# twmitchel/FieldConv

Measured on AMD Instinct MI355X. Metric: FieldConv fwd+bwd Medges/s (20k verts, k=32, C=48, M=2), higher is better.
Workload: dtype f32 (complex64 in/out; contractions on f16 MFMA with every operand split into two halves, fp32 accumulate)

## Files before the change

fieldconv_amd/_env.py:

```python
import os

SWITCHES = {
    'FC_MFMA': 'f32: fp32-MFMA contractions throughout; f16: single halves (reduced precision); default: split halves',
    'FC_RING': '0: frequency-major forward kernels for every mesh size; 2: ring-major ones for every size',
    'FC_GROUP_SPLIT': '0: the backward data kernel never runs the two frequency groups of a tile as separate work items; 2 (development): wherever legal',
    'FC_RING_COMPACT': '0: no compact LDS plans (aliased partials, half-size record chunks) for the ring-major forward kernel',
    'FC_RING_HALVES': '0: no half tiles in the last round of the ring-major forward kernel',
    'FC_HALF_TILES': '0: no half tiles in the frequency-major kernels; 2: half tiles in the backward kernels too',
    'FC_BWD_STREAM': '0: the data / filter kernel pair on large meshes too, instead of the H-streaming arrangement (gather + stream + gx kernels)',
    'FC_FILTER2': '0: the LDS-staged half-precision filter-gradient kernel instead of the register-fed one',
    'FC_SPLIT_FINISH': '1: partial sums and parameter-gradient chain as two launches',
    'FC_EDGE_PARTS_MAX': 'cap (log2) on the number of workgroups that share a tile on small meshes',
    'FC_ECHO_WPV': 'wavefronts per vertex in the ECHO descriptor kernels (1, 2 or 4)',
    'FC_STAMP_KERNEL': 'data | filter | stream: which backward kernel writes in-kernel time stamps (tools/stamps.py)',
    'FC_DEBUG': 'forward kernels: skip phases (WRONG RESULTS; refused by bench.py)',
    'FC_DEBUG_BWD': 'backward kernels: skip phases (bit 0 walk, bit 1 gxt product, bit 2 gW product, bit 3 H stores) (WRONG RESULTS; refused by bench.py)',
    'FC_LIN_DIRECT': '0: TangentLin on small meshes through the LDS-staged kernel instead of the direct one',
    'FC_DEBUG_RG': "ECHOBlock head's grouped GEMM: 1 no products, 2 no loads, 4 no staging (WRONG RESULTS; refused by bench.py)",
    'FC_DEBUG_RP': 'finishing launch: 1 no partial loads, 2 no parameter-gradient chain (WRONG RESULTS; refused by bench.py)',
    'FIELDCONV_DEV': '1: load libfieldconv_hip_dev.so (the library switches above exist there only; one of them set without this raises)',
    'FIELDCONV_HIP_LIB': 'path of a prebuilt libfieldconv_hip.so (development variants, fieldconv_amd.build.build_variant)',
    'FIELDCONV_DENSE': '1: FCPrecomp stencils through the dense-stencil kernels',
    'FIELDCONV_NO_GEO': '1: 64-byte factored records in the forward pass instead of geometric ones',
    'FIELDCONV_TORCH_GRAPH': '1: support graph built with torch ops instead of fc_graph_build',
    'FIELDCONV_NO_EDGE_SPLIT': '1: no edge split on small meshes',
    'FIELDCONV_EAGER_STENCIL': '1: FCPrecomp returns the dense (E,R,F) tensor',
    'FIELDCONV_NO_FUSED_EPILOGUE': '1: residual add and modReLU as separate operators',
    'FIELDCONV_SEPARATE_CALLS': '1: one foreign call per kernel instead of fc_forward_params / fc_backward_all',
    'FIELDCONV_CPP_NODES': '0: the block-level autograd nodes in Python (fieldconv_amd/blocks.py) instead of the C++ ones (fc_torch_nodes.so)',
    'FIELDCONV_ECHO_TAIL': "0: ECHOBlock's dense tail as torch's own Linear / ReLU autograd nodes instead of one node; aten: one node composed "
                           "of ATen GEMMs instead of the native head (fc_echo_head_*)",
    'FIELDCONV_BLOCK_CALLS': '0: FCResNetBlock / ECHOBlock / LiftBlock composed of per-operator autograd nodes instead of the block-level entry points',
    'BENCH_BACKEND': 'gloo: several ranks share a device (test rigs); default nccl (= RCCL)',
    'BENCH_FORCE_DIST': '1: run the partitioned / data-parallel code path with one rank',
    'BENCH_FORWARD_OVERLAP': '1: interior targets under the forward halo exchange',
    'BENCH_NO_OVERLAP': '1: gradient halo exchange not overlapped with the filter-gradient kernel',
    'BENCH_GRAPH_STEP': '1: the partitioned step captured in one HIP graph',
}

TEST_SWITCHES = {
    'FC_FULL_MODES': '1: tests/test_gpu_modes.py sweeps every development switch instead of the eight kernel-family / arithmetic modes',
    'FC_FUZZ_SHAPES': 'number of shapes in the seeded sweep against the oracle (default 40)',
    'FC_FUZZ_SEED': 'seed of that sweep',
    'FC_FUZZ_WIDE': '1: the sweep also draws layers wider than 64 channels and (n_rings, band_limit) pairs outside the compiled set',
    'FC_DIST_TEST_DEVICE': 'cuda: the distributed test worker runs the HIP kernels (two gloo ranks on one GPU)',
    'FC_DIST_OVERLAP': '0: the distributed test worker without forward / backward overlap',
    'FC_DIST_PLAN_ONLY': '1: the distributed test worker checks partition and halo plan at config-4 size only',
    'FC_DIST_CONFIG4': '1: the distributed GPU test worker runs config 4\'s per-rank size (20 000 owned vertices per rank)',
}

LIBRARY_SWITCHES = ('FC_BWD_STREAM', 'FC_RING', 'FC_GROUP_SPLIT', 'FC_RING_COMPACT', 'FC_RING_HALVES', 'FC_HALF_TILES', 'FC_FILTER2', 'FC_SPLIT_FINISH',
                    'FC_EDGE_PARTS_MAX', 'FC_ECHO_WPV', 'FC_STAMP_KERNEL', 'FC_DEBUG', 'FC_DEBUG_BWD', 'FC_DEBUG_RP', 'FC_DEBUG_RG', 'FC_LIN_DIRECT')

PREFIXES = ('FC_', 'FIELDCONV_', 'BENCH_')
WRONG_RESULTS = ('FC_DEBUG', 'FC_DEBUG_BWD', 'FC_DEBUG_RP', 'FC_DEBUG_RG')


def active(environ=None):
    environ = os.environ if environ is None else environ
    return {k: environ[k] for k in sorted(SWITCHES) if k in environ}


def unknown(environ=None):
    environ = os.environ if environ is None else environ
    return sorted(k for k in environ if k.startswith(PREFIXES) and k not in SWITCHES and k not in TEST_SWITCHES)
```

fieldconv_amd/csrc/fc_backward.hip:

```cpp
#include <stdio.h>
#include "fc_backward_kernels.hpp"
#include "fc_backward_stream.hpp"

namespace fc {

template <int T>
__global__ __launch_bounds__(kThreads) void fc_backward_filter_kernel(
    const float2* __restrict__ gx_, const float* __restrict__ hdump, float2* __restrict__ ggwp ,
    const BwdArgs a, const int F, const int B) {
    extern __shared__ __attribute__((aligned(16))) char smem[];
    const MmaGeom& mg = a.g;
    const int KD = a.KD, KP = mg.KP, IP = mg.MP, I = a.I;
    float* const slab0 = reinterpret_cast<float*>(smem);
    float* const xtr = slab0 + 2 * a.slab_stride;
    float* const xts = xtr + IP * kXtStride;
    float* const xtd = xts + IP * kXtStride;

    const int tid = threadIdx.x;
    const int lane = tid & 63;
    const int wave = __builtin_amdgcn_readfirstlane(tid >> 6);
    const int f = blockIdx.y;
    const int m = f - B;
    const int fr = lane & 15, fq = lane >> 4;

// ... 424 lines not shown
            if ((a.dbg & 32) && wave < mg.NMT) {
                const lds_f16* arow = img + fr * KSI + 8 * fq;
                const lds_f16* brow = img0 + (buf ^ 1) * kTile * KSI + fr * KSI + 8 * fq;
                f32x4 xr = {0.f, 0.f, 0.f, 0.f}, xi = xr;
                for (int kb = 0; kb < KP / 32; ++kb) {
                    const u32x4 arh = *reinterpret_cast<lds_u32x4*>(arow + kb * 32), arl = *reinterpret_cast<lds_u32x4*>(arow + kb * 32 + KP);
                    const u32x4 aih = *reinterpret_cast<lds_u32x4*>(arow + kb * 32 + 2 * KP), ail = *reinterpret_cast<lds_u32x4*>(arow + kb * 32 + 3 * KP);
                    const u32x4 brh = *reinterpret_cast<lds_u32x4*>(brow + kb * 32), brl = *reinterpret_cast<lds_u32x4*>(brow + kb * 32 + KP);
                    const u32x4 bih = *reinterpret_cast<lds_u32x4*>(brow + kb * 32 + 2 * KP), bil = *reinterpret_cast<lds_u32x4*>(brow + kb * 32 + 3 * KP);
                    xr = mfma32h(arh, brh, xr); xr = mfma32h(arh, brl, xr); xr = mfma32h(arl, brh, xr);
                    xr = mfma32h(aih, bih, xr); xr = mfma32h(aih, bil, xr); xr = mfma32h(ail, bih, xr);
                    xi = mfma32h(aih, brh, xi); xi = mfma32h(aih, brl, xi); xi = mfma32h(ail, brh, xi);
                    xi = mfma32h(arh, bih, xi); xi = mfma32h(arh, bil, xi); xi = mfma32h(arl, bih, xi);
                }
                const size_t cap = (size_t)gridDim.x * F * KP * IP;
                const size_t base = (((size_t)tile * F + f) * mg.NMT + wave) * 256 % (cap - 256);
#pragma unroll
                for (int jj = 0; jj < 4; ++jj) ggwp[base + (4 * fq + jj) * 16 + fr] = make_float2(xr[jj] * it, xi[jj] * it);
            }
        }
    
    };
    int buf = 0;
    for (int tile = blockIdx.x; tile < a.ntiles; tile += tile_step, buf ^= 1) {
        one_tile(tile, ahead0, buf);
        stamp(3);
    }
    stamp(30);
    stamp.realtime(31);

#pragma unroll
    for (int n = 0; n < T; ++n) {
        if (gw_h[n] >= 0) {
#pragma unroll
            for (int jj = 0; jj < 4; ++jj) {
                const int k = gw_h[n] + 4 * fq + jj;
                const int i = i0 + fr;
                ggwp[(((size_t)blockIdx.x * F + f) * KP + k) * IP + i] = make_float2(gre[n][jj], gim[n][jj]);
            }
        }
    }
}

__global__ void fc_reduce_gw_kernel(const float2* __restrict__ gwp, float2* __restrict__ gw, int P, int F, int R,
                                    int O, int I, int KP, int IP, int pairs ) {
    const int idx = blockIdx.x * blockDim.x + threadIdx.x;
    const int total = F * R * O * I;
    if (idx >= total) return;
    const int i = idx % I;
    const int k = (idx / I) % (R * O);
    const int f = idx / (I * R * O);
    float2 s = make_float2(0.f, 0.f);
    const size_t stride = (size_t)F * KP * IP;
    const float2* src = gwp + ((size_t)f * KP + k) * IP + i;
    int p = 0;
    for (; p + 8 <= P; p += 8) {
        float2 v[8];
#pragma unroll
        for (int u = 0; u < 8; ++u) v[u] = src[(size_t)(p + u) * stride];
#pragma unroll
        for (int u = 0; u < 8; ++u) { s.x += v[u].x; s.y += v[u].y; }
    }
    for (; p < P; ++p) {
        const float2 v = src[(size_t)p * stride];
        s.x += v.x;
        s.y += v.y;
    }
    const float sc = 1.f / (float)F;
    int r = k / O, o = k - r * O;
    if (pairs == 2) {
        o = k / R;
        r = k - o * R;
    } else if (pairs && k < (R >> 1) * 2 * O) {
        const int pr = k / (2 * O), rem = k - pr * 2 * O;
        r = 2 * pr + (rem & 1);
        o = rem >> 1;
    }
    gw[(((size_t)o * I + i) * R + r) * F + f] = make_float2(s.x * sc, s.y * sc);
}

template <int R, int B>
static int launch_gather(const float2* gy, const float* rec, const fc_csr* g, const float* wpk, char* hrec, const StreamArgs& a,
                         const StreamPlan& p, hipStream_t stream) {
    auto kern = fc_backward_gather_kernel<R, B>;
    const size_t lds = (size_t)kWaves * kRingChunks * 1024;
    const int grid = p.ntiles < num_cus() ? p.ntiles : num_cus();
    hipLaunchKernelGGL(kern, dim3(grid), dim3(kThreads), lds, stream, gy, rec, g->rowptr, g->runs, wpk, hrec, a);
    return hipGetLastError() == hipSuccess ? FC_OK : FC_ERR_LAUNCH;
}

template <int T, int KPT = 0, int IT = 0>
static int launch_stream(const float2* x, const char* hrec, const float* wpk, float2* gwp, float2* gxt, const StreamArgs& a,
                         const StreamPlan& p, hipStream_t stream) {
    auto kern = fc_backward_stream_kernel<T, KPT, IT>;
    static bool lds_ok[kMaxDevices] = {};
    if (!allow_full_lds(reinterpret_cast<const void*>(kern), p.lds, lds_ok)) return FC_ERR_LAUNCH;
    hipLaunchKernelGGL(kern, dim3(p.P, p.FS), dim3(kThreads), p.lds, stream, x, hrec, wpk, gwp, gxt, a);
    return hipGetLastError() == hipSuccess ? FC_OK : FC_ERR_LAUNCH;
}

int backward_stream_impl(const float* x, const float* gy, const float* rec, const fc_csr* g, const float* wpk, float* gx, void* ws,
                         size_t ws_bytes, const fc_dims* d, hipStream_t stream, int stages) {
    const StreamPlan p = plan_stream(d, halves_of(d), true);
    if (!p.ok) return FC_ERR_UNSUPPORTED;
    if (!ws || ws_bytes < p.hrec_bytes + p.gwp_bytes + p.gxt_bytes + p.wst_bytes) return FC_ERR_WORKSPACE;
    StreamArgs a = make_stream_args(d, p);
    char* hrec = static_cast<char*>(ws);
    a.wst = reinterpret_cast<uint32_t*>(hrec + p.hrec_bytes + p.gwp_bytes + p.gxt_bytes);
    float2* gwp = reinterpret_cast<float2*>(hrec + p.hrec_bytes);
    float2* gxt = reinterpret_cast<float2*>(hrec + p.hrec_bytes + p.gwp_bytes);
    const float2* x2 = reinterpret_cast<const float2*>(x);
    int rc = FC_ERR_UNSUPPORTED;
    if (stages & 1) {
        const float2* gy2 = reinterpret_cast<const float2*>(gy);
#define FC_GATHER_CASE(RR, BB) if (d->R == RR && d->B == BB) rc = launch_gather<RR, BB>(gy2, rec, g, wpk, hrec, a, p, stream);
        FC_GATHER_CASE(2, 1) FC_GATHER_CASE(4, 1) FC_GATHER_CASE(6, 1) FC_GATHER_CASE(8, 1)
        FC_GATHER_CASE(2, 2) FC_GATHER_CASE(4, 2) FC_GATHER_CASE(6, 2) FC_GATHER_CASE(8, 2)
        FC_GATHER_CASE(2, 3) FC_GATHER_CASE(4, 3) FC_GATHER_CASE(6, 3) FC_GATHER_CASE(8, 3)
#undef FC_GATHER_CASE
        if (rc != FC_OK) return rc;
    }
    if (!(stages & 2)) return FC_OK;
    if (p.T == 6 && p.KPS == 288 && d->I == 48) rc = launch_stream<6, 288, 48>(x2, hrec, wpk, gwp, gxt, a, p, stream);
    else if (p.T == 6 && p.KPS == 192 && d->I == 64) rc = launch_stream<6, 192, 64>(x2, hrec, wpk, gwp, gxt, a, p, stream);
    else if (p.T <= 2) rc = launch_stream<2>(x2, hrec, wpk, gwp, gxt, a, p, stream);
    else if (p.T <= 4) rc = launch_stream<4>(x2, hrec, wpk, gwp, gxt, a, p, stream);
    else rc = launch_stream<6>(x2, hrec, wpk, gwp, gxt, a, p, stream);
    if (rc != FC_OK || (stages & 4)) return rc;
    const size_t count = (size_t)d->N * d->I;
    const dim3 grid((unsigned)((count + 255) / 256));
    float2* gx2 = reinterpret_cast<float2*>(gx);
    if (d->B == 1) hipLaunchKernelGGL(fc_backward_gx_kernel<1>, grid, dim3(256), 0, stream, x2, gxt, gx2, count, p.KS);
    else if (d->B == 2) hipLaunchKernelGGL(fc_backward_gx_kernel<2>, grid, dim3(256), 0, stream, x2, gxt, gx2, count, p.KS);
    else hipLaunchKernelGGL(fc_backward_gx_kernel<3>, grid, dim3(256), 0, stream, x2, gxt, gx2, count, p.KS);
    return hipGetLastError() == hipSuccess ? FC_OK : FC_ERR_LAUNCH;
}

bool backward_streams(const fc_dims* d, bool factored) { return plan_stream(d, halves_of(d), factored).ok; }

bool backward_fits(const fc_dims* d) { return plan_backward(d, halves_of(d)).ok_factored; }

size_t backward_workspace_bytes(const fc_dims* d) {
    const BwdPlan p = plan_backward(d, halves_of(d));
    const size_t pair = p.hdump_bytes + p.gwp_bytes + p.gxp_bytes + 256;
    const StreamPlan sp = plan_stream(d, halves_of(d), true);
    const size_t stream = sp.ok ? sp.hrec_bytes + sp.gwp_bytes + sp.gxt_bytes + sp.wst_bytes + 256 : 0;
    return pair > stream ? pair : stream;
}

template <int T>
static int launch_backward_filter(const float2* x, const float* hdump, float2* gwp, const BwdArgs& a, const BwdPlan& p,
                                  const fc_dims* d, hipStream_t stream) {
    static const bool half2 = !(dev_env("FC_FILTER2") && atoi(dev_env("FC_FILTER2")) == 0);
    static bool ok_half2[kMaxDevices] = {}, ok_half[kMaxDevices] = {}, ok_f32[kMaxDevices] = {};
    if (p.fhalf && half2) {
        const size_t lds2 = (size_t)(2 * kTile * filter_image_stride(p.KP) + 2 * 6 * p.IP * kXbStride + 8) * sizeof(_Float16) + 16;
        static bool ok_half2h[kMaxDevices] = {};
        if (a.dump_halves) {
            if (!allow_full_lds(reinterpret_cast<const void*>(fc_backward_filter_half2_kernel<T, true>), lds2, ok_half2h)) return FC_ERR_LAUNCH;
            hipLaunchKernelGGL((fc_backward_filter_half2_kernel<T, true>), dim3(p.P, p.F), dim3(kThreads), lds2, stream, x, hdump, gwp, a, p.F,
                               d->B, d->R * d->O);
        } else {
            if (!allow_full_lds(reinterpret_cast<const void*>(fc_backward_filter_half2_kernel<T, false>), lds2, ok_half2)) return FC_ERR_LAUNCH;
            hipLaunchKernelGGL((fc_backward_filter_half2_kernel<T, false>), dim3(p.P, p.F), dim3(kThreads), lds2, stream, x, hdump, gwp, a, p.F,
                               d->B, d->R * d->O);
        }
    } else if (p.fhalf) {
        if (!allow_full_lds(reinterpret_cast<const void*>(fc_backward_filter_half_kernel<T>), p.lds_filter, ok_half)) return FC_ERR_LAUNCH;
        hipLaunchKernelGGL(fc_backward_filter_half_kernel<T>, dim3(p.P, p.F), dim3(kThreads), p.lds_filter, stream, x, hdump, gwp, a,
                           p.F, d->B, d->R * d->O);
    } else {
        if (!allow_full_lds(reinterpret_cast<const void*>(fc_backward_filter_kernel<T>), p.lds_filter, ok_f32)) return FC_ERR_LAUNCH;
        hipLaunchKernelGGL(fc_backward_filter_kernel<T>, dim3(p.P, p.F), dim3(kThreads), p.lds_filter, stream, x, hdump, gwp, a, p.F,
                           d->B);
    }
    return hipGetLastError() == hipSuccess ? FC_OK : FC_ERR_LAUNCH;
}

int backward_filter_impl(const float* x, void* ws, size_t ws_bytes, const fc_dims* d, hipStream_t stream, bool factored) {
    if (backward_streams(d, factored)) return FC_OK;
    const BwdPlan p = plan_backward(d, halves_of(d));
    if (!p.ok) return FC_ERR_UNSUPPORTED;
    if (!ws || ws_bytes < p.hdump_bytes + p.gwp_bytes) return FC_ERR_WORKSPACE;
    const BwdArgs a = make_args(d, p);
    const float* hdump = reinterpret_cast<const float*>(ws);
    float2* gwp = reinterpret_cast<float2*>(static_cast<char*>(ws) + p.hdump_bytes);
    const float2* x2 = reinterpret_cast<const float2*>(x);
    int need = (p.ngw + kWaves - 1) / kWaves;
    if (p.fhalf) {
        const int per_col = kWaves / p.g.NMT, row_tiles = p.KP / 16;
        need = (row_tiles + per_col - 1) / per_col;
    }
    if (need <= 2) return launch_backward_filter<2>(x2, hdump, gwp, a, p, d, stream);
    if (need <= 4) return launch_backward_filter<4>(x2, hdump, gwp, a, p, d, stream);
    if (need <= 6) return launch_backward_filter<6>(x2, hdump, gwp, a, p, d, stream);
    if (need <= kMaxGwTiles) return launch_backward_filter<kMaxGwTiles>(x2, hdump, gwp, a, p, d, stream);
    return FC_ERR_UNSUPPORTED;
}

void describe_backward(const fc_dims* d, int records, char* buf, size_t n) {
    {
        const StreamPlan sp = plan_stream(d, halves_of(d), records != 0);
        if (sp.ok) {
            snprintf(buf, n, "fc_backward_gather_kernel<records,split-f16> tiles=%d; fc_backward_stream_kernel (H once for gxt and gW: %d gxt + %d gW "
                     "wavefronts, W_f in registers, records by LDS-DMA) grid=%dx%d; fc_backward_gx_kernel; module parameters: "
                     "fc_backward_finish_params (sum of the partials + parameter chain) in one launch; explicit filter: fc_backward_finish; cus=%d",
                     sp.ntiles, sp.G, sp.NW, sp.P, sp.FS, num_cus());
            return;
        }
    }
    const BwdPlan p = plan_backward(d, halves_of(d));
    const char* mode = halves_of(d) == 2 ? "split-f16" : halves_of(d) == 1 ? "f16" : "f32";
    static const bool staged = [] { const char* e = dev_env("FC_FILTER2"); return e && atoi(e) == 0; }();
    static const bool split_finish = [] { const char* e = dev_env("FC_SPLIT_FINISH"); return e && atoi(e) != 0; }();
    const int gx_parts = (1 << p.parts_log2) * (p.gsplit ? 2 : 1);
    char fin[320];
    if (split_finish)
        snprintf(fin, sizeof(fin), "%sfc_backward_finish + fc_filter_param_grads (two launches: the split-finish development switch)",
                 gx_parts > 1 ? "fc_sum_parts_kernel (the partial gx arrays), " : "");
    else
        snprintf(fin, sizeof(fin), "module parameters: fc_backward_finish_params (sum of the partials + parameter chain%s, + a fused modReLU's "
                 "bias-gradient sum when given) in one launch; explicit filter: %sfc_backward_finish",
                 gx_parts > 1 ? " + sum of the partial gx arrays" : "", gx_parts > 1 ? "fc_sum_parts_kernel, " : "");
    snprintf(buf, n, "fc_backward_data_kernel<%s,%s> tiles=%d parts=%d%s; %s; %s; cus=%d", records ? "records" : "dense rows", mode, p.ntiles,
             1 << p.parts_log2, p.gsplit ? " (the two frequency groups of a tile as separate work items)" : "",
             p.fhalf ? (staged ? "fc_backward_filter_half_kernel (LDS-staged slabs)" : "fc_backward_filter_half2_kernel (register-fed rows)")
                     : "fc_backward_filter_kernel (fp32 MFMA)",
             fin, num_cus());
}

int backward_finish_impl(float* gw_eff, void* ws, size_t ws_bytes, const fc_dims* d, hipStream_t stream, bool factored) {
    {
        const StreamPlan sp = plan_stream(d, halves_of(d), factored);
        if (sp.ok) {
            if (!ws || ws_bytes < sp.hrec_bytes + sp.gwp_bytes) return FC_ERR_WORKSPACE;
            const float2* gwp = reinterpret_cast<const float2*>(static_cast<char*>(ws) + sp.hrec_bytes);
            const int total = sp.F * d->R * d->O * d->I;
            hipLaunchKernelGGL(fc_reduce_gw_kernel, dim3((total + 255) / 256), dim3(256), 0, stream, gwp, reinterpret_cast<float2*>(gw_eff),
                               sp.P, sp.F, d->R, d->O, d->I, sp.KP, sp.IP, 2);
            return hipGetLastError() == hipSuccess ? FC_OK : FC_ERR_LAUNCH;
        }
    }
    const BwdPlan p = plan_backward(d, halves_of(d));
    if (!p.ok) return FC_ERR_UNSUPPORTED;
    if (!ws || ws_bytes < p.hdump_bytes + p.gwp_bytes) return FC_ERR_WORKSPACE;
    const float2* gwp = reinterpret_cast<const float2*>(static_cast<char*>(ws) + p.hdump_bytes);
    const int total = p.F * d->R * d->O * d->I;
    hipLaunchKernelGGL(fc_reduce_gw_kernel, dim3((total + 255) / 256), dim3(256), 0, stream, gwp,
                       reinterpret_cast<float2*>(gw_eff), p.P, p.F, d->R, d->O, d->I, p.KP, p.IP, p.gd.split != 0 ? 1 : 0);
    return hipGetLastError() == hipSuccess ? FC_OK : FC_ERR_LAUNCH;
}

int backward_finish_params_impl(float* gw_eff, void* ws, size_t ws_bytes, const fc_dims* d, const fc_filter_params* fp, hipStream_t stream,
                                int o0, int i0, int Ifull, float* gx_deferred, bool factored, const float* x_for_gx) {
    {
        const StreamPlan sp = plan_stream(d, halves_of(d), factored);
        if (sp.ok) {
            if (!ws || ws_bytes < sp.hrec_bytes + sp.gwp_bytes + sp.gxt_bytes) return FC_ERR_WORKSPACE;
            const float* gwp = reinterpret_cast<const float*>(static_cast<char*>(ws) + sp.hrec_bytes);
            const bool ride = gx_deferred && x_for_gx;
            const float* gxt = reinterpret_cast<const float*>(static_cast<char*>(ws) + sp.hrec_bytes + sp.gwp_bytes);
            return reduce_param_grads_impl(gwp, (size_t)sp.F * sp.KP * sp.IP, (size_t)sp.IP, (size_t)sp.KP * sp.IP, (size_t)d->R * sp.IP, false, sp.P,
                                           gw_eff, fp->zonal, fp->spherical, fp->phase, fp->ftype, fp->g_zonal, fp->g_spherical, fp->g_phase, d,
                                           stream, o0, i0, Ifull, fp->bias_partials, fp->bias_nparts, fp->g_bias, ride ? gxt : nullptr,
                                           ride ? gx_deferred : nullptr, (size_t)d->N * d->I, 0, ride ? -(d->B + 4 * (sp.KS - 1)) : 0, ride ? x_for_gx : nullptr);
        }
    }
    const BwdPlan p = plan_backward(d, halves_of(d));
    if (!p.ok) return FC_ERR_UNSUPPORTED;
    if (!ws || ws_bytes < p.hdump_bytes + p.gwp_bytes) return FC_ERR_WORKSPACE;
    const float* gwp = reinterpret_cast<const float*>(static_cast<char*>(ws) + p.hdump_bytes);
    const int gx_nparts = gx_deferred ? (1 << p.parts_log2) << p.gsplit : 1;
    const float* gxp = gx_nparts > 1 ? reinterpret_cast<const float*>(static_cast<char*>(ws) + p.hdump_bytes + p.gwp_bytes) : nullptr;
    return reduce_param_grads_impl(gwp, (size_t)p.F * p.KP * p.IP, (size_t)d->O * p.IP, (size_t)p.KP * p.IP, (size_t)p.IP, p.gd.split != 0, p.P, gw_eff,
                                   fp->zonal, fp->spherical, fp->phase, fp->ftype, fp->g_zonal, fp->g_spherical, fp->g_phase, d, stream, o0,
                                   i0, Ifull, fp->bias_partials, fp->bias_nparts, fp->g_bias, gxp, gx_deferred, (size_t)d->N * d->I,
                                   p.gx_part_stride, gx_nparts);
}

#define FC_BWD_DATA_ARGS const float*, const float*, const float*, const fc_csr*, const float*, float*, void*, size_t, const fc_dims*, bool, hipStream_t, bool
template int backward_data_impl_mode<false>(FC_BWD_DATA_ARGS);
extern template int backward_data_impl_mode<true>(FC_BWD_DATA_ARGS);

int backward_data_impl(const float* x, const float* gy, const float* sten, const fc_csr* g, const float* wpk, float* gx,
                       void* ws, size_t ws_bytes, const fc_dims* d, bool factored, hipStream_t stream, bool defer_gx_sum) {
    if (backward_streams(d, factored)) return backward_stream_impl(x, gy, sten, g, wpk, gx, ws, ws_bytes, d, stream, defer_gx_sum ? 7 : 3);
    return halves_of(d) ? backward_data_impl_mode<true>(x, gy, sten, g, wpk, gx, ws, ws_bytes, d, factored, stream, defer_gx_sum)
                        : backward_data_impl_mode<false>(x, gy, sten, g, wpk, gx, ws, ws_bytes, d, factored, stream, defer_gx_sum);
}

// ... 2 lines not shown
```

fieldconv_amd/csrc/fc_backward_stream.hpp:

```cpp
#pragma once
#include <stdlib.h>
#include "fc_backward_kernels.hpp"

namespace fc {

constexpr int kStreamUnits = 4;
constexpr int kStreamPartStride = 2 * kTile + 4;

struct StreamPlan {
    bool ok;
    int F, KP, IP, NMT, KST, KSI, NU, G, NW, T, ntiles, P, nslots;
    int KS;
    int FS, KPS;
    int NG;
    int img_bytes;
    int rec_bytes;
    size_t lds;
    size_t hrec_bytes, gwp_bytes, gxt_bytes, wst_bytes;
    int nt_dump;
};

struct StreamArgs {
    int N, I, O, R, F, B;
    int KP, IP, NMT, KST, KSI, G, NW, ntiles, P, nslots;
    int KS;
    int img_bytes, rec_bytes;
    int wKI, wKP;
    int nt_dump;
    uint32_t* wst;
    unsigned long long* stamps;
    int dbg;
};

inline StreamPlan plan_stream(const fc_dims* d, int halves, bool factored) {
    StreamPlan p = {};
    p.ok = false;
    static const bool off = [] { const char* e = dev_env("FC_BWD_STREAM"); return e && atoi(e) == 0; }();
    if (off || !factored || halves != 2 || d->N <= 0) return p;
    const int R = d->R, O = d->O, I = d->I;
    p.F = 2 * d->B + 1;
    if (R < 2 || R > 8 || (R & 1) || (R * O) % 32 != 0 || I > 64 || O > 64 || d->B < 1 || d->B > 3) return p;
    p.NG = (p.F * R + 31) / 32;
    if (p.NG > 2) return p;
    p.KP = R * O;
    p.IP = round_up(I, 16);
    p.NMT = p.IP / 16;
    bool fits = false;
    for (p.KS = 1; p.KS <= 2 && !fits; ++p.KS) {
        if (p.KS == 2 && ((O & 1) || (p.KP / 2) % 32 != 0)) break;
        p.KPS = p.KP / p.KS;
        p.KST = p.KPS / 32;
        if (p.KST < 3) break;
        p.NU = p.NMT * p.KST;
        p.G = (p.NU + kStreamUnits - 1) / kStreamUnits;
        p.NW = kWaves - p.G;
        if (p.NW < p.NMT || p.NW < 8 || p.G < 1) continue;
        const int row_tiles = p.KPS / 16, min_ct_waves = p.NW / p.NMT;
        p.T = (row_tiles + min_ct_waves - 1) / min_ct_waves;
        fits = p.T <= 6;
        if (fits) break;
    }
    if (!fits) return p;
    p.FS = p.F * p.KS;
    p.KSI = filter_image_stride(p.KPS);
    p.nslots = p.G + p.NMT - 1;
    p.ntiles = (d->N + kTile - 1) / kTile;
    const int cus = num_cus();
    if (4 * p.ntiles < 3 * cus) return p;
    p.P = cus / p.FS;
    if (p.P < 1) p.P = 1;
    p.img_bytes = kTile * p.KSI * 2;
    p.rec_bytes = round_up(p.img_bytes + 2 * kTile * 4, 1024);
    if (I & 1) return p;
    p.lds = (size_t)2 * p.rec_bytes + (size_t)2 * 4 * p.IP * kXbStride * 2 + (size_t)3 * kTile * I * 8 + 4 * 64 * 4 + 2 * 8 * 64 * 4 +
            2 * 64 * 4 + (size_t)2 * p.nslots * kTile * kStreamPartStride * 4;
    if (kTile * I * 8 > kWaves * 1024 - 1024) return p;
    if ((size_t)d->N * I * 8 >= ((size_t)1 << 32)) return p;
    if (p.lds > kMaxLds) return p;
    p.hrec_bytes = (size_t)p.ntiles * p.FS * p.rec_bytes + 1024;
    p.gwp_bytes = (size_t)p.P * p.F * p.KP * p.IP * sizeof(float2);
    p.gxt_bytes = (size_t)p.FS * d->N * I * sizeof(float2);
    p.wst_bytes = (size_t)p.FS * p.G * 4 * kStreamUnits * kWave * 16;
    p.nt_dump = p.hrec_bytes > ((size_t)192 << 20) ? 1 : 0;
    p.ok = true;
    return p;
}

inline StreamArgs make_stream_args(const fc_dims* d, const StreamPlan& p) {
    StreamArgs a;
    a.N = d->N; a.I = d->I; a.O = d->O; a.R = d->R; a.F = p.FS; a.B = d->B; a.KS = p.KS;
    a.KP = p.KPS; a.IP = p.IP; a.NMT = p.NMT; a.KST = p.KST; a.KSI = p.KSI; a.G = p.G; a.NW = p.NW; a.ntiles = p.ntiles; a.P = p.P;
    a.nslots = p.nslots;
    a.img_bytes = p.img_bytes; a.rec_bytes = p.rec_bytes;
    const MmaGeom gw = make_mma_geom(d->I, d->R, d->O, 2);
    a.wKI = gw.KI; a.wKP = gw.KP;
    a.nt_dump = p.nt_dump;
    a.wst = nullptr;
    static const int dbg = [] { const char* e = dev_env("FC_DEBUG_BWD"); return e ? atoi(e) : 0; }();
    a.dbg = dbg;
    static const bool stamp_me = [] { const char* e = dev_env("FC_STAMP_KERNEL"); return e && e[0] == 's'; }();
    a.stamps = stamp_me ? debug_stamp_buffer() : nullptr;
    return a;
}

typedef uint32_t u32x3 __attribute__((ext_vector_type(3)));

template <int R, bool NT>
__device__ __forceinline__ void store_plane_row(uint32_t* dst, const uint32_t (&w)[R / 2]) {
    if constexpr (R == 2) {
        if (NT) __builtin_nontemporal_store(w[0], dst); else *dst = w[0];
    } else if constexpr (R == 4) {
        typedef u32x2 __attribute__((aligned(4))) u2;
        const u32x2 v = {w[0], w[1]};
        if (NT) __builtin_nontemporal_store(v, reinterpret_cast<u2*>(dst)); else *reinterpret_cast<u2*>(dst) = v;
    } else if constexpr (R == 6) {
        typedef u32x3 __attribute__((aligned(4))) u3;
        const u32x3 v = {w[0], w[1], w[2]};
        if (NT) __builtin_nontemporal_store(v, reinterpret_cast<u3*>(dst)); else *reinterpret_cast<u3*>(dst) = v;
    } else {
        typedef u32x4 __attribute__((aligned(4))) u4;
        const u32x4 v = {w[0], w[1], w[2], w[3]};
        if (NT) __builtin_nontemporal_store(v, reinterpret_cast<u4*>(dst)); else *reinterpret_cast<u4*>(dst) = v;
    }
}

template <int R, int B>
__global__ __launch_bounds__(kThreads) void fc_backward_gather_kernel(
    const float2* __restrict__ ggy, const float* __restrict__ gsten, const int32_t* __restrict__ growptr,
    const int32_t* __restrict__ gruns, const float* __restrict__ gwpk, char* __restrict__ hrec, const StreamArgs a) {
    constexpr int F = 2 * B + 1;
    static_assert(F * R <= 64 && (R & 1) == 0, "at most two walks per vertex, an even ring count");
    constexpr int NG = (F * R + 31) / 32;
    constexpr int FG = (F + NG - 1) / NG;
    constexpr int RECF = factored_record_floats(B);
    constexpr int LOG_CR = factored_log_chunk_records(B);
    constexpr int CR = 1 << LOG_CR;
    constexpr int NR = kRingChunks;
    extern __shared__ __attribute__((aligned(16))) char smem[];
    const int tid = threadIdx.x;
    const int lane = tid & 63;
    const int wave = __builtin_amdgcn_readfirstlane(tid >> 6);
    float* const ring = reinterpret_cast<float*>(smem) + wave * NR * 256;
    const int O = a.O;
    const int ol = lane < O ? lane : 0;

    auto dma_chunk = [&](const int first, const int ch) {
        const float* src = gsten + ((size_t)first + ((size_t)ch << LOG_CR)) * RECF + lane * 4;
        __builtin_amdgcn_global_load_lds((gptr_t)src, (lptr_t)(ring + (ch & (NR - 1)) * 256), 16, 0, 0);
    };
    auto slot_range = [&](const int tile, int& b, int& e, int (&run)[R]) {
        b = 0;
        e = 0;
#pragma unroll
        for (int q = 0; q < R; ++q) run[q] = 0;
        const int j = tile * kTile + wave;
        if (tile < a.ntiles && j < a.N) {
            b = growptr[j];
            e = growptr[j + 1];
#pragma unroll
            for (int q = 0; q < R; ++q) run[q] = gruns[(size_t)j * kRunStride + q];
        }
    };
    auto rec_ptr = [&](const int s) {
        if constexpr (CR * RECF == 256) return ring + ((s * RECF) & (NR * 256 - 1));
        else return ring + ((s >> LOG_CR) & (NR - 1)) * 256 + (s & (CR - 1)) * RECF;
    };

    const int grid = gridDim.x;
    int beg = 0, end = 0, ro[R];
    {
        slot_range(first_tile_of_block(), beg, end, ro);
        const int nch = (end - beg + CR - 1) >> LOG_CR;
        for (int ch = 0; ch < min(nch, NR); ++ch) dma_chunk(beg, ch);
    }
    const int OH = O / a.KS;
    const int half = (lane >= OH && a.KS == 2) ? 1 : 0;
    const int lane_in_half = lane - half * OH;
    for (int tile = first_tile_of_block(); tile < a.ntiles; tile += grid) {
        int nbeg = 0, nend = 0, nro[R];
        slot_range(tile + grid, nbeg, nend, nro);
        const int nslots = end - beg;
        const int nch = (nslots + CR - 1) >> LOG_CR;
        char* const rec0 = hrec + (size_t)tile * a.F * a.rec_bytes;
        const int row_off = wave * a.KSI * 2 + lane_in_half * R * 2;

        static_for<0, NG>([&](auto gc) {
            constexpr int GI = decltype(gc)::value;
            constexpr int F0 = GI * FG;
            constexpr int NF = (F - F0) < FG ? (F - F0) : FG;
            f32x2 h[R][NF];
#pragma unroll
            for (int r = 0; r < R; ++r)
#pragma unroll
                for (int f = 0; f < NF; ++f) h[r][f] = f32x2{0.f, 0.f};

            float2 ga = make_float2(0.f, 0.f), gb = ga;
            if (nslots > 0) {
                asm volatile("s_waitcnt vmcnt(0)" ::: "memory");
                const int d0 = __float_as_int(rec_ptr(0)[3]);
                const int d1 = __float_as_int(rec_ptr(min(1, nslots - 1))[3]);
                ga = gather_row(ggy, d0, 8u * O, 8u * ol);
                gb = gather_row(ggy, d1, 8u * O, 8u * ol);
            }
            auto slot = [&](auto qc, const int s, float2& gcur) {
                constexpr int Q = decltype(qc)::value;
                const float* rp = rec_ptr(s);
                const f32x4 head = *reinterpret_cast<const f32x4*>(rp);
                const int d2 = __float_as_int(rec_ptr(min(s + 2, nslots - 1))[3]);
                const f32x2 gv = f32x2{gcur.x, gcur.y};
                gcur = gather_row(ggy, d2, 8u * O, 8u * ol);
                const f32x2 w0v = f32x2{head.y, head.y}, w1v = f32x2{head.z, head.z};
                f32x2 ph[NF], z[NF];
#pragma unroll
                for (int f = 0; f < NF; ++f) {
                    ph[f] = *reinterpret_cast<const f32x2*>(rp + 4 + 2 * (F0 + f));
                    z[f] = cmul_conj_pk_step1(gv, ph[f]);
                }
#pragma unroll
                for (int f = 0; f < NF; ++f) z[f] = cmul_conj_pk_step2(gv, ph[f], z[f]);
#pragma unroll
                for (int f = 0; f < NF; ++f) h[Q][f] = __builtin_elementwise_fma(w0v, z[f], h[Q][f]);
#pragma unroll
                for (int f = 0; f < NF; ++f) h[Q + 1][f] = __builtin_elementwise_fma(w1v, z[f], h[Q + 1][f]);
            };
            if (!(kDevSwitches && (a.dbg & 1))) {
                static_for<0, R - 1>([&](auto qc) {
                    constexpr int Q = decltype(qc)::value;
                    int s = ro[Q];
                    const int run_end = (Q + 1 < R - 1) ? ro[Q + 1] : nslots;
                    while (s < run_end) {
                        const int m = s & (CR - 1);
                        if (m == 0 && s > 0) {
                            const int ch = s >> LOG_CR;
                            asm volatile("s_waitcnt vmcnt(0)" ::: "memory");
                            if (ch - 1 + NR < nch) dma_chunk(beg, ch - 1 + NR);
                        }
                        const int stop = min(run_end, s - m + CR);
                        if ((s & 1) && s < stop) {
                            slot(qc, s, gb);
                            ++s;
                        }
                        for (; s + 1 < stop; s += 2) {
                            slot(qc, s, ga);
                            slot(qc, s + 1, gb);
                        }
                        if (s < stop) {
                            slot(qc, s, ga);
                            ++s;
                        }
                    }
                });
            }
            {
                asm volatile("s_waitcnt vmcnt(0) lgkmcnt(0)" ::: "memory");
                if constexpr (GI + 1 < NG) {
                    for (int ch = 0; ch < min(nch, NR); ++ch) dma_chunk(beg, ch);
                } else {
                    const int nnch = (nend - nbeg + CR - 1) >> LOG_CR;
                    for (int ch = 0; ch < min(nnch, NR); ++ch) dma_chunk(nbeg, ch);
                }
            }

            float mx = 0.f;
#pragma unroll
            for (int r = 0; r < R; ++r)
#pragma unroll
                for (int f = 0; f < NF; ++f) mx = fmaxf(mx, fmaxf(fabsf(h[r][f].x), fabsf(h[r][f].y)));
            mx = wave_max_nonneg(mx);
            float scale, inv_scale;
            split_scale(mx, scale, inv_scale);
            if (mx == 0.f) inv_scale = 0.f;
            auto rows = [&](auto nt_c) {
                constexpr bool NT = decltype(nt_c)::value;
#pragma unroll
                for (int f = 0; f < NF; ++f) {
                    uint32_t hi[R], lo[R];
#pragma unroll
                    for (int r = 0; r < R; ++r) {
                        f16x2 h2, l2;
                        split_halves2(h[r][f], scale, h2, l2);
                        hi[r] = __builtin_bit_cast(uint32_t, h2);
                        lo[r] = __builtin_bit_cast(uint32_t, l2);
                    }
                    constexpr uint32_t kLow = 0x05040100u, kHigh = 0x07060302u;
                    uint32_t p0[R / 2], p1[R / 2], p2[R / 2], p3[R / 2];
#pragma unroll
                    for (int dd = 0; dd < R / 2; ++dd) {
                        p0[dd] = __builtin_amdgcn_perm(hi[2 * dd + 1], hi[2 * dd], kLow);
                        p1[dd] = __builtin_amdgcn_perm(lo[2 * dd + 1], lo[2 * dd], kLow);
                        p2[dd] = __builtin_amdgcn_perm(hi[2 * dd + 1], hi[2 * dd], kHigh);
                        p3[dd] = __builtin_amdgcn_perm(lo[2 * dd + 1], lo[2 * dd], kHigh);
                    }
                    char* const recf = rec0 + (size_t)((F0 + f) * a.KS + half) * a.rec_bytes;
                    if (lane < O && !(kDevSwitches && (a.dbg & 8))) {
                        char* const dst = recf + row_off;
                        store_plane_row<R, NT>(reinterpret_cast<uint32_t*>(dst), p0);
                        store_plane_row<R, NT>(reinterpret_cast<uint32_t*>(dst + a.KP * 2), p1);
                        store_plane_row<R, NT>(reinterpret_cast<uint32_t*>(dst + a.KP * 4), p2);
                        store_plane_row<R, NT>(reinterpret_cast<uint32_t*>(dst + a.KP * 6), p3);
                    }
                    if (lane_in_half == 0 && lane < O) {
                        float* tail = reinterpret_cast<float*>(recf + a.img_bytes);
                        tail[wave] = scale;
                        tail[kTile + wave] = inv_scale;
                    }
                }
            };
            if (a.nt_dump && !(kDevSwitches && (a.dbg & 32))) rows(std::true_type{}); else rows(std::false_type{});
        });
        beg = nbeg;
        end = nend;
#pragma unroll
        for (int q = 0; q < R; ++q) ro[q] = nro[q];
    }

    {
        const int total = a.F * a.G * kStreamUnits * 4 * kWave;
        const int NU = a.NMT * a.KST;
        const size_t plane_sz = (size_t)a.IP * a.wKP;
        const uint16_t* const img0 = reinterpret_cast<const uint16_t*>(gwpk + a.IP);
        for (int e = blockIdx.x * kThreads + tid; e < total; e += gridDim.x * kThreads) {
            const int ln = e & 63, pl = (e >> 6) & 3, ui = (e >> 8) % kStreamUnits, fg = e / (kStreamUnits * 4 * kWave);
            const int g_ = fg % a.G, sl = fg / a.G;
            const int f_ = sl / a.KS, k0 = (sl - f_ * a.KS) * a.KP;
            const int fr_ = ln & 15, fq_ = ln >> 4;
            const int u = min(g_ * kStreamUnits + ui, NU - 1);
            const int mt = u / a.KST, kb = u - mt * a.KST;
            const int row = (mt * 16 + fr_) * 32;
            const uint16_t* const img = img0 + ((size_t)f_ * 4 + pl) * plane_sz;
            int o = (k0 + kb * 32 + 8 * fq_) / R, r = k0 + kb * 32 + 8 * fq_ - o * R;
            uint32_t v[4];
#pragma unroll
            for (int jj = 0; jj < 4; ++jj) {
                uint32_t pr[2];
#pragma unroll
                for (int e2 = 0; e2 < 2; ++e2) {
                    const int kk = r * a.wKI + o;
                    pr[e2] = img[(size_t)(kk >> 5) * a.IP * 32 + row + (kk & 31)];
                    if (++r == R) { r = 0; ++o; }
                }
                v[jj] = pr[0] | (pr[1] << 16);
            }
            *reinterpret_cast<u32x4*>(a.wst + (size_t)e * 4) = u32x4{v[0], v[1], v[2], v[3]};
        }
    }
}

template <int T, int KPT = 0, int IT = 0>
__global__ __launch_bounds__(kThreads) void fc_backward_stream_kernel(
    const float2* __restrict__ gx_, const char* __restrict__ hrec, const float* __restrict__ gwpk,
    float2* __restrict__ ggwp , float2* __restrict__ ggxt , const StreamArgs a) {
    extern __shared__ __attribute__((aligned(16))) char smem[];
    const int KP = KPT ? KPT : a.KP, I = IT ? IT : a.I, IP = IT ? round_up(IT, 16) : a.IP, KSI = KPT ? filter_image_stride(KPT) : a.KSI;
    const int F = a.F, N = a.N;
    const int xplane = IP * kXbStride;
    const int xrs = I * 8;
    const int xtile = kTile * xrs;
    lds_f16* const xb0 = (lds_f16*)(smem + 2 * a.rec_bytes);
    char* const xrow0 = smem + 2 * a.rec_bytes + 2 * 4 * xplane * 2;
    float* const tail0 = reinterpret_cast<float*>(xrow0 + 3 * xtile);
    float* const pmax0 = tail0 + 4 * 64;
    float* const tinv0 = pmax0 + 2 * 8 * 64;
    float* const part0 = tinv0 + 2 * 64;
    const int part_floats = a.nslots * kTile * kStreamPartStride;

    const int tid = threadIdx.x;
    const int lane = tid & 63;
    const int wave = __builtin_amdgcn_readfirstlane(tid >> 6);
    const int f = blockIdx.y;
    const int m = f / a.KS - a.B;
    const int fr = lane & 15, fq = lane >> 4;
    const bool is_gxt = wave < a.G;
    const int op_pair = (wave >= a.G && wave - a.G < 8) ? wave - a.G : -1;
    const int red_idx = wave < 6 && wave < a.G ? wave : -1;
    const int n_red = a.G < 6 ? a.G : 6;

    const int nrec = ((int)blockIdx.x < a.ntiles) ? (a.ntiles - (int)blockIdx.x + a.P - 1) / a.P : 0;
    const int npieces = a.rec_bytes >> 10;
    const int nxp = (xtile + 1023) >> 10;
    const bool rev = kDevSwitches && (a.dbg & 64);
    auto tile_of = [&](const int k) { return (int)blockIdx.x + (rev ? nrec - 1 - k : k) * a.P; };
    const uint32_t lane16 = lane * 16;
    auto dma_piece = [&](const int q, const int krec, const int kx) {
        if (q < npieces) {
            if (krec < nrec) {
                const char* src = hrec + ((size_t)tile_of((kDevSwitches && (a.dbg & 16)) ? 0 : krec) * F + f) * a.rec_bytes;
                lds_dma16_saddr(src + q * 1024, lane16, smem + (krec & 1) * a.rec_bytes + q * 1024);
            }
        } else if (kx < nrec) {
            const int tile = tile_of(kx);
            const int xq = q - npieces;
            if (xq < nxp) {
                const uint32_t voff = min((uint32_t)tile * (uint32_t)xtile + (uint32_t)xq * 1024u + lane16, (uint32_t)N * (uint32_t)xrs - 16u);
                const int left = xtile - xq * 1024;
                if (left >= 1024) lds_dma16_saddr(gx_, voff, xrow0 + (kx % 3) * xtile + xq * 1024);
                else lds_dma16_saddr_lanes(gx_, voff, xrow0 + (kx % 3) * xtile + xq * 1024, (1ull << (left / 16)) - 1ull);
            } else {
                lds_dma4_saddr(hrec + ((size_t)tile * F + f) * a.rec_bytes + a.img_bytes, lane * 4, tail0 + (kx & 3) * 64);
            }
        }
    };
    auto requests = [&](const int krec, const int kx, const int nd) {
        if (wave < nd)
            for (int q = wave; q < npieces + nxp + 1; q += nd) dma_piece(q, krec, kx);
    };
    auto pair_max = [&](const int k) {
        if (k >= nrec || op_pair < 0) return;
        const char* rows = xrow0 + (k % 3) * xtile + (2 * op_pair) * xrs;
        const float* tl = tail0 + (k & 3) * 64 + kTile + 2 * op_pair;
        const int lc = lane < I ? lane : 0;
        const float2 x0 = *reinterpret_cast<const float2*>(rows + lc * 8), x1 = *reinterpret_cast<const float2*>(rows + xrs + lc * 8);
        const float i0_ = tl[0], i1_ = tl[1];
        const float m0 = (x0.x * x0.x + x0.y * x0.y) * (i0_ * i0_), m1 = (x1.x * x1.x + x1.y * x1.y) * (i1_ * i1_);
        pmax0[((k & 1) * 8 + op_pair) * 64 + lane] = lane < I ? fmaxf(m0, m1) : 0.f;
    };
    const int pm_ = m < 0 ? -m : m;
    auto pair_rows = [&](const int k) {
        if (k >= nrec || op_pair < 0) return;
        lds_f16* const xb = xb0 + (k & 1) * 4 * xplane;
        const char* rows = xrow0 + (k % 3) * xtile + (2 * op_pair) * xrs;
        const float* tl = tail0 + (k & 3) * 64 + kTile + 2 * op_pair;
        const float* pm = pmax0 + (k & 1) * 8 * 64 + lane;
        const int lc = lane < I ? lane : 0;
        float pv[8];
#pragma unroll
        for (int j = 0; j < 8; ++j) pv[j] = pm[j * 64];
        float2 xv[2];
        float inv[2];
// ... 284 lines not shown
```

Before: 1863.

## Launch backward gather kernel as residency-bounded 4-wavefront workgroups when registers allow

The gather kernel of the H-streaming backward pass is templated on wavefronts per workgroup and a minimum-residency launch bound. When the compiled 4-wave variant has no spills and few enough registers, it launches five such workgroups per CU instead of one 16-wave workgroup per CU. Work items become groups of 4 vertices inside a 16-row tile, and the record row and half offsets are recomputed from that. The aim is more resident wavefronts and finer load balancing to hide gather latency, at the cost of tighter register limits and smaller DMA ring LDS per workgroup. An environment switch can force either variant.

```diff
diff --git a/fieldconv_amd/_env.py b/fieldconv_amd/_env.py
--- a/fieldconv_amd/_env.py
+++ b/fieldconv_amd/_env.py
@@ -8,6 +8,7 @@
     'FC_RING_HALVES': '0: no half tiles in the last round of the ring-major forward kernel',
     'FC_HALF_TILES': '0: no half tiles in the frequency-major kernels; 2: half tiles in the backward kernels too',
     'FC_BWD_STREAM': '0: the data / filter kernel pair on large meshes too, instead of the H-streaming arrangement (gather + stream + gx kernels)',
+    'FC_GATHER_WPG': '16 / 4: the gather kernel of the H-streaming arrangement as one 16-wavefront workgroup per CU / as five 4-wavefront ones, whatever its registers say',
     'FC_FILTER2': '0: the LDS-staged half-precision filter-gradient kernel instead of the register-fed one',
     'FC_SPLIT_FINISH': '1: partial sums and parameter-gradient chain as two launches',
     'FC_EDGE_PARTS_MAX': 'cap (log2) on the number of workgroups that share a tile on small meshes',
@@ -49,7 +50,7 @@
     'FC_DIST_CONFIG4': '1: the distributed GPU test worker runs config 4\'s per-rank size (20 000 owned vertices per rank)',
 }
 
-LIBRARY_SWITCHES = ('FC_BWD_STREAM', 'FC_RING', 'FC_GROUP_SPLIT', 'FC_RING_COMPACT', 'FC_RING_HALVES', 'FC_HALF_TILES', 'FC_FILTER2', 'FC_SPLIT_FINISH',
+LIBRARY_SWITCHES = ('FC_BWD_STREAM', 'FC_GATHER_WPG', 'FC_RING', 'FC_GROUP_SPLIT', 'FC_RING_COMPACT', 'FC_RING_HALVES', 'FC_HALF_TILES', 'FC_FILTER2', 'FC_SPLIT_FINISH',
                     'FC_EDGE_PARTS_MAX', 'FC_ECHO_WPV', 'FC_STAMP_KERNEL', 'FC_DEBUG', 'FC_DEBUG_BWD', 'FC_DEBUG_RP', 'FC_DEBUG_RG', 'FC_LIN_DIRECT')
 
 PREFIXES = ('FC_', 'FIELDCONV_', 'BENCH_')
diff --git a/fieldconv_amd/csrc/fc_backward.hip b/fieldconv_amd/csrc/fc_backward.hip
--- a/fieldconv_amd/csrc/fc_backward.hip
+++ b/fieldconv_amd/csrc/fc_backward.hip
@@ -530,10 +530,13 @@
 template <int R, int B>
 static int launch_gather(const float2* gy, const float* rec, const fc_csr* g, const float* wpk, char* hrec, const StreamArgs& a,
                          const StreamPlan& p, hipStream_t stream) {
-    auto kern = fc_backward_gather_kernel<R, B>;
-    const size_t lds = (size_t)kWaves * kRingChunks * 1024;
-    const int grid = p.ntiles < num_cus() ? p.ntiles : num_cus();
-    hipLaunchKernelGGL(kern, dim3(grid), dim3(kThreads), lds, stream, gy, rec, g->rowptr, g->runs, wpk, hrec, a);
+    const size_t lds = (size_t)p.gwpg * kRingChunks * 1024;
+    if (p.gwpg == kGatherSmallWaves)
+        hipLaunchKernelGGL((fc_backward_gather_kernel<R, B, kGatherSmallWaves, kGatherSmallResidency>), dim3(p.ggrid), dim3(kGatherSmallWaves * kWave),
+                           lds, stream, gy, rec, g->rowptr, g->runs, wpk, hrec, a);
+    else
+        hipLaunchKernelGGL((fc_backward_gather_kernel<R, B, kWaves, kWaves / 4>), dim3(p.ggrid), dim3(kThreads), lds, stream, gy, rec, g->rowptr,
+                           g->runs, wpk, hrec, a);
     return hipGetLastError() == hipSuccess ? FC_OK : FC_ERR_LAUNCH;
 }
 
@@ -650,10 +653,10 @@
     {
         const StreamPlan sp = plan_stream(d, halves_of(d), records != 0);
         if (sp.ok) {
-            snprintf(buf, n, "fc_backward_gather_kernel<records,split-f16> tiles=%d; fc_backward_stream_kernel (H once for gxt and gW: %d gxt + %d gW "
+            snprintf(buf, n, "fc_backward_gather_kernel<records,split-f16> tiles=%d (%d workgroups of %d wavefronts, %d per SIMD); fc_backward_stream_kernel (H once for gxt and gW: %d gxt + %d gW "
                      "wavefronts, W_f in registers, records by LDS-DMA) grid=%dx%d; fc_backward_gx_kernel; module parameters: "
                      "fc_backward_finish_params (sum of the partials + parameter chain) in one launch; explicit filter: fc_backward_finish; cus=%d",
-                     sp.ntiles, sp.G, sp.NW, sp.P, sp.FS, num_cus());
+                     sp.ntiles, sp.ggrid, sp.gwpg, sp.gwaves, sp.G, sp.NW, sp.P, sp.FS, num_cus());
             return;
         }
     }
diff --git a/fieldconv_amd/csrc/fc_backward_stream.hpp b/fieldconv_amd/csrc/fc_backward_stream.hpp
--- a/fieldconv_amd/csrc/fc_backward_stream.hpp
+++ b/fieldconv_amd/csrc/fc_backward_stream.hpp
@@ -13,6 +13,8 @@
     int KS;
     int FS, KPS;
     int NG;
+    int gwpg, gwaves;
+    int ggrid;
     int img_bytes;
     int rec_bytes;
     size_t lds;
@@ -31,6 +33,10 @@
     unsigned long long* stamps;
     int dbg;
 };
+
+constexpr int kGatherSmallWaves = 4;
+constexpr int kGatherSmallResidency = 5;
+inline void plan_gather(const fc_dims* d, StreamPlan& p);
 
 inline StreamPlan plan_stream(const fc_dims* d, int halves, bool factored) {
     StreamPlan p = {};
@@ -82,6 +88,7 @@
     p.gxt_bytes = (size_t)p.FS * d->N * I * sizeof(float2);
     p.wst_bytes = (size_t)p.FS * p.G * 4 * kStreamUnits * kWave * 16;
     p.nt_dump = p.hrec_bytes > ((size_t)192 << 20) ? 1 : 0;
+    plan_gather(d, p);
     p.ok = true;
     return p;
 }
@@ -124,8 +131,8 @@
     }
 }
 
-template <int R, int B>
-__global__ __launch_bounds__(kThreads) void fc_backward_gather_kernel(
+template <int R, int B, int WPG, int MINW>
+__global__ __launch_bounds__(WPG * kWave, MINW) void fc_backward_gather_kernel(
     const float2* __restrict__ ggy, const float* __restrict__ gsten, const int32_t* __restrict__ growptr,
     const int32_t* __restrict__ gruns, const float* __restrict__ gwpk, char* __restrict__ hrec, const StreamArgs a) {
     constexpr int F = 2 * B + 1;
@@ -145,16 +152,18 @@
     const int ol = lane < O ? lane : 0;
 
     auto dma_chunk = [&](const int first, const int ch) {
-        const float* src = gsten + ((size_t)first + ((size_t)ch << LOG_CR)) * RECF + lane * 4;
+        uint32_t lane_off = lane;
+        asm volatile("" : "+v"(lane_off));
+        const char* src = reinterpret_cast<const char*>(gsten + ((size_t)first + ((size_t)ch << LOG_CR)) * RECF) + lane_off * 16u;
         __builtin_amdgcn_global_load_lds((gptr_t)src, (lptr_t)(ring + (ch & (NR - 1)) * 256), 16, 0, 0);
     };
-    auto slot_range = [&](const int tile, int& b, int& e, int (&run)[R]) {
+    auto slot_range = [&](const int item, int& b, int& e, int (&run)[R]) {
         b = 0;
         e = 0;
 #pragma unroll
         for (int q = 0; q < R; ++q) run[q] = 0;
-        const int j = tile * kTile + wave;
-        if (tile < a.ntiles && j < a.N) {
+        const int j = item * WPG + wave;
+        if (j < a.N) {
             b = growptr[j];
             e = growptr[j + 1];
 #pragma unroll
@@ -166,7 +175,8 @@
         else return ring + ((s >> LOG_CR) & (NR - 1)) * 256 + (s & (CR - 1)) * RECF;
     };
 
-    const int grid = gridDim.x;
+    static_assert(kTile % WPG == 0, "whole groups per tile");
+    const int grid = gridDim.x, nitems = a.ntiles * (kTile / WPG);
     int beg = 0, end = 0, ro[R];
     {
         slot_range(first_tile_of_block(), beg, end, ro);
@@ -174,15 +184,13 @@
         for (int ch = 0; ch < min(nch, NR); ++ch) dma_chunk(beg, ch);
     }
     const int OH = O / a.KS;
-    const int half = (lane >= OH && a.KS == 2) ? 1 : 0;
-    const int lane_in_half = lane - half * OH;
-    for (int tile = first_tile_of_block(); tile < a.ntiles; tile += grid) {
+    for (int item = first_tile_of_block(); item < nitems; item += grid) {
         int nbeg = 0, nend = 0, nro[R];
-        slot_range(tile + grid, nbeg, nend, nro);
+        slot_range(item + grid, nbeg, nend, nro);
+        const int j = item * WPG + wave, tile = j >> 4, row = j & (kTile - 1);
         const int nslots = end - beg;
         const int nch = (nslots + CR - 1) >> LOG_CR;
         char* const rec0 = hrec + (size_t)tile * a.F * a.rec_bytes;
-        const int row_off = wave * a.KSI * 2 + lane_in_half * R * 2;
 
         static_for<0, NG>([&](auto gc) {
             constexpr int GI = decltype(gc)::value;
@@ -270,6 +278,12 @@
             float scale, inv_scale;
             split_scale(mx, scale, inv_scale);
             if (mx == 0.f) inv_scale = 0.f;
+            int ln = lane;
+            asm volatile("" : "+v"(ln));
+            const int half = (ln >= OH && a.KS == 2) ? 1 : 0;
+            const int lane_in_half = ln - half * OH;
+            const uint32_t half_off = (uint32_t)half * (uint32_t)a.rec_bytes;
+            const uint32_t row_off = half_off + (uint32_t)(row * a.KSI * 2 + lane_in_half * R * 2);
             auto rows = [&](auto nt_c) {
                 constexpr bool NT = decltype(nt_c)::value;
 #pragma unroll
@@ -291,18 +305,18 @@
                         p2[dd] = __builtin_amdgcn_perm(hi[2 * dd + 1], hi[2 * dd], kHigh);
                         p3[dd] = __builtin_amdgcn_perm(lo[2 * dd + 1], lo[2 * dd], kHigh);
                     }
-                    char* const recf = rec0 + (size_t)((F0 + f) * a.KS + half) * a.rec_bytes;
-                    if (lane < O && !(kDevSwitches && (a.dbg & 8))) {
+                    char* const recf = rec0 + (size_t)((F0 + f) * a.KS) * a.rec_bytes;
+                    if (ln < O && !(kDevSwitches && (a.dbg & 8))) {
                         char* const dst = recf + row_off;
                         store_plane_row<R, NT>(reinterpret_cast<uint32_t*>(dst), p0);
                         store_plane_row<R, NT>(reinterpret_cast<uint32_t*>(dst + a.KP * 2), p1);
                         store_plane_row<R, NT>(reinterpret_cast<uint32_t*>(dst + a.KP * 4), p2);
                         store_plane_row<R, NT>(reinterpret_cast<uint32_t*>(dst + a.KP * 6), p3);
                     }
-                    if (lane_in_half == 0 && lane < O) {
-                        float* tail = reinterpret_cast<float*>(recf + a.img_bytes);
-                        tail[wave] = scale;
-                        tail[kTile + wave] = inv_scale;
+                    if (lane_in_half == 0 && ln < O) {
+                        float* tail = reinterpret_cast<float*>(recf + half_off + (uint32_t)a.img_bytes);
+                        tail[row] = scale;
+                        tail[kTile + row] = inv_scale;
                     }
                 }
             };
@@ -319,7 +333,7 @@
         const int NU = a.NMT * a.KST;
         const size_t plane_sz = (size_t)a.IP * a.wKP;
         const uint16_t* const img0 = reinterpret_cast<const uint16_t*>(gwpk + a.IP);
-        for (int e = blockIdx.x * kThreads + tid; e < total; e += gridDim.x * kThreads) {
+        for (int e = (blockIdx.x * WPG + wave) * kWave + lane; e < total; e += gridDim.x * (WPG * kWave)) {
             const int ln = e & 63, pl = (e >> 6) & 3, ui = (e >> 8) % kStreamUnits, fg = e / (kStreamUnits * 4 * kWave);
             const int g_ = fg % a.G, sl = fg / a.G;
             const int f_ = sl / a.KS, k0 = (sl - f_ * a.KS) * a.KP;
@@ -344,6 +358,36 @@
             *reinterpret_cast<u32x4*>(a.wst + (size_t)e * 4) = u32x4{v[0], v[1], v[2], v[3]};
         }
     }
+}
+
+template <int R, int B>
+inline bool gather_fits_small() {
+    static const bool fits = [] {
+        hipFuncAttributes at;
+        const void* fn = reinterpret_cast<const void*>(fc_backward_gather_kernel<R, B, kGatherSmallWaves, kGatherSmallResidency>);
+        if (hipFuncGetAttributes(&at, fn) != hipSuccess) {
+            (void)hipGetLastError();
+            return false;
+        }
+        return at.localSizeBytes == 0 && at.numRegs <= (512 / kGatherSmallResidency) / 8 * 8;
+    }();
+    return fits;
+}
+
+inline void plan_gather(const fc_dims* d, StreamPlan& p) {
+    bool small = false;
+#define FC_GATHER_CASE(RR, BB) if (d->R == RR && d->B == BB) small = gather_fits_small<RR, BB>();
+    FC_GATHER_CASE(2, 1) FC_GATHER_CASE(4, 1) FC_GATHER_CASE(6, 1) FC_GATHER_CASE(8, 1)
+    FC_GATHER_CASE(2, 2) FC_GATHER_CASE(4, 2) FC_GATHER_CASE(6, 2) FC_GATHER_CASE(8, 2)
+    FC_GATHER_CASE(2, 3) FC_GATHER_CASE(4, 3) FC_GATHER_CASE(6, 3) FC_GATHER_CASE(8, 3)
+#undef FC_GATHER_CASE
+    static const int forced = [] { const char* e = dev_env("FC_GATHER_WPG"); return e ? atoi(e) : 0; }();
+    if (forced == kWaves) small = false;
+    if (forced == kGatherSmallWaves) small = true;
+    p.gwpg = small ? kGatherSmallWaves : kWaves;
+    p.gwaves = small ? kGatherSmallResidency : kWaves / 4;
+    const int nitems = p.ntiles * (kTile / p.gwpg), places = num_cus() * (small ? kGatherSmallResidency : 1);
+    p.ggrid = nitems < places ? nitems : places;
 }
 
 template <int T, int KPT = 0, int IT = 0>
```

Measured after the change: 1900, median of 6. 1.02x the previous value.
